# imkaywu/MVSKit

Measured on AMD Instinct MI355X. Metric: patches/s (propagate+optim iteration), 12-view 1080p, higher is better.
Workload: dtype f32

## Files before the change

mvskit_amd/csrc/mvs_engine.cpp:

```cpp
#include <hip/hip_runtime.h>
#include <dlfcn.h>
#include <rccl/rccl.h>

#include <algorithm>
#include <climits>
#include <cmath>
#include <cstdio>
#include <cstdlib>
#include <cstring>
#include <string>
#include <vector>

#include "mvskit_engine.h"
#include "mvs_kernels.h"
#include "mvs_types.h"

static_assert(sizeof(mvs_patch) == sizeof(DPatch), "mvs_patch and DPatch must be the same bytes");
static_assert((MVS_LISTCAP == 16 || MVS_LISTCAP == 32 || MVS_LISTCAP == 64) && MVS_LISTCAP <= MVS_MAXI && MVS_MAX_IMAGES == MVS_MAXI, "limits out of sync");

namespace {
thread_local std::string g_err;

#define HIPCHK(expr)                                                                                       \
    do {                                                                                                   \
        hipError_t _e = (expr);                                                                            \
        if (_e != hipSuccess) {                                                                            \
            g_err = std::string(#expr) + ": " + hipGetErrorString(_e);                                     \
            return MVS_ERR_HIP;                                                                            \
        }                                                                                                  \
    } while (0)

template <typename T> struct DevBuf {
    T* p = nullptr;
    int64_t cap = 0;
    bool headroom = false;
    DevBuf() = default;
    DevBuf(const DevBuf&) = delete;
    DevBuf(DevBuf&& o) noexcept : p(o.p), cap(o.cap), headroom(o.headroom) { o.p = nullptr; o.cap = 0; }
    ~DevBuf() { release(); }
    void swap(DevBuf& o) { std::swap(p, o.p); std::swap(cap, o.cap); }
    int ensure(int64_t n) {
        if (n <= cap) return MVS_OK;
        const int64_t exact = std::max<int64_t>(n, 16);
        int64_t want = (p && headroom) ? exact + exact / 2 : exact;
        T* q = nullptr;
        hipError_t e = hipMalloc((void**)&q, (size_t)want * sizeof(T));
        if (e != hipSuccess && want > exact) { (void)hipGetLastError(); want = exact; e = hipMalloc((void**)&q, (size_t)want * sizeof(T)); }
        if (e != hipSuccess && p) {
            (void)hipGetLastError();
            (void)hipFree(p); p = nullptr; cap = 0;
            e = hipMalloc((void**)&q, (size_t)want * sizeof(T));
        }
        if (e != hipSuccess) { (void)hipGetLastError(); g_err = std::string("hipMalloc: ") + hipGetErrorString(e); return MVS_ERR_HIP; }
        if (p) (void)hipFree(p);
        p = q; cap = want;
        return MVS_OK;
    }
    void release() { if (p) (void)hipFree(p); p = nullptr; cap = 0; }
};

namespace misc {
constexpr int stage_counter = 0;
constexpr int fill_evals = 1;
constexpr int neighbor_retry = 4;
constexpr int sweep_retry = 5;
constexpr int geo_bad = 6;
constexpr int group_edges = 7;
constexpr int trim_parts = 8;
constexpr int trim_nparts = 256;
constexpr int words = trim_parts + trim_nparts;
}
namespace fstat {
constexpr int neighbor_parts = 0;
constexpr int neighbor_cycles = 4096;
constexpr int exact_evals = 4112;
constexpr int words = exact_evals + 2048;
}

struct Rccl {
    void* h = nullptr;
    ncclResult_t (*GetUniqueId)(ncclUniqueId*) = nullptr;
    ncclResult_t (*CommInitRank)(ncclComm_t*, int, ncclUniqueId, int) = nullptr;
    ncclResult_t (*CommDestroy)(ncclComm_t) = nullptr;
    ncclResult_t (*CommCount)(const ncclComm_t, int*) = nullptr;
    ncclResult_t (*CommUserRank)(const ncclComm_t, int*) = nullptr;
    ncclResult_t (*AllGather)(const void*, void*, size_t, ncclDataType_t, ncclComm_t, hipStream_t) = nullptr;
    ncclResult_t (*Broadcast)(const void*, void*, size_t, ncclDataType_t, int, ncclComm_t, hipStream_t) = nullptr;
    ncclResult_t (*GroupStart)() = nullptr;
    ncclResult_t (*GroupEnd)() = nullptr;
    const char* (*GetErrorString)(ncclResult_t) = nullptr;
    bool ok = false;
};
Rccl& rccl() {
    static Rccl r;
    static bool tried = false;
    if (tried) return r;
    tried = true;
    if (const char* over = getenv("MVS_CCL_LIBRARY")) {
        if (*over) { r.h = dlopen(over, RTLD_NOW | RTLD_LOCAL); if (!r.h) return r; }
    }
    const char* names[] = {"librccl.so", "librccl.so.1"};
    for (const char* n : names) if (!r.h) r.h = dlopen(n, RTLD_NOW | RTLD_NOLOAD);
    const char* paths[] = {"/opt/rocm/lib/librccl.so.1", "librccl.so.1", "librccl.so"};
    for (const char* n : paths) if (!r.h) r.h = dlopen(n, RTLD_NOW | RTLD_LOCAL);
    if (!r.h) return r;
#define MVS_SYM(field, name) r.field = reinterpret_cast<decltype(r.field)>(dlsym(r.h, name))
    MVS_SYM(GetUniqueId, "ncclGetUniqueId"); MVS_SYM(CommInitRank, "ncclCommInitRank"); MVS_SYM(CommDestroy, "ncclCommDestroy");
    MVS_SYM(AllGather, "ncclAllGather"); MVS_SYM(Broadcast, "ncclBroadcast"); MVS_SYM(GroupStart, "ncclGroupStart");
    MVS_SYM(GroupEnd, "ncclGroupEnd"); MVS_SYM(GetErrorString, "ncclGetErrorString");
    MVS_SYM(CommCount, "ncclCommCount"); MVS_SYM(CommUserRank, "ncclCommUserRank");
#undef MVS_SYM
    r.ok = r.GetUniqueId && r.CommInitRank && r.CommDestroy && r.AllGather && r.Broadcast && r.GroupStart && r.GroupEnd && r.GetErrorString;
    return r;
}
#define NCCLCHK(expr)                                                                                      \
    do {                                                                                                   \
        ncclResult_t _r = (expr);                                                                          \
        if (_r != ncclSuccess) {                                                                           \
            g_err = std::string(#expr) + ": " + rccl().GetErrorString(_r);                                 \
            return MVS_ERR_HIP;                                                                            \
        }                                                                                                  \
    } while (0)

// ... 1006 lines not shown
    int64_t nj = 0;
    const bool ranged = e->cfg.shard_count > 1;
    for (int v = ranged ? 0 : e->cfg.view_begin; v < e->cfg.nviews; v += ranged ? 1 : e->cfg.view_stride) {
        a.sweep_views[a.nsweep_views] = v;
        a.job_base[a.nsweep_views] = (int32_t)nj;
        ++a.nsweep_views;
        nj += (int64_t)((e->hviews[v].gw + 1) / 2) * e->hviews[v].gh;
    }
    a.njobs = nj;
    a.job_lo = 0; a.job_hi = nj;
    if (ranged) {
        const int split_mode = getenv("MVS_SPLIT_PROXY") ? atoi(getenv("MVS_SPLIT_PROXY")) : 2;
        const int N = e->cfg.shard_count, R = e->cfg.shard_index;
        std::vector<int32_t> cuts(N + 1, -1);
        int64_t total_work = 0;
        if (split_mode > 0 && nj > 0) {
            const DParams p0 = current_params(e);
            int shift = 0;
            while ((((int64_t)3 * e->prm.cap * e->prm.max_propag * 32 * nj) >> shift) + nj >= (int64_t)INT32_MAX) ++shift;
            mvsk_job_work(p0, a, split_mode, shift, e->job_cnt.p, st);
            mvsk_exclusive_scan(e->job_cnt.p, e->job_base_scan.p, nj, reinterpret_cast<int32_t*>(e->scan_tmp.p), st);
            if (int r = e->tmp_i.ensure(N + 1)) return r;
            HIPCHK(hipMemsetAsync(e->tmp_i.p, 0xff, (size_t)(N + 1) * sizeof(int32_t), st));
            mvsk_job_cuts(e->job_base_scan.p, nj, N, e->tmp_i.p, st);
            int32_t tw = 0;
            HIPCHK(hipMemcpyAsync(cuts.data(), e->tmp_i.p, (size_t)(N + 1) * sizeof(int32_t), hipMemcpyDeviceToHost, st));
            HIPCHK(hipMemcpyAsync(&tw, e->job_base_scan.p + nj, sizeof tw, hipMemcpyDeviceToHost, st));
            HIPCHK(hipStreamSynchronize(st));
            total_work = tw;
        }
        cuts[0] = 0; cuts[N] = (int32_t)nj;
        for (int r = 1; r < N; ++r) {
            if (total_work <= 0 || cuts[r] < 0) cuts[r] = (int32_t)(nj * r / N);
            cuts[r] = std::max(cuts[r], cuts[r - 1]);
        }
        a.job_lo = cuts[R];
        a.job_hi = cuts[R + 1];
        HIPCHK(hipMemsetAsync(e->job_nstage.p, 0, (size_t)nj * sizeof(int32_t), st));
    }
    a.staging = e->staging.p; a.staging_cap = e->staging.cap;
    a.stage_counter = e->misc.p + misc::stage_counter;
    a.job_stage = e->job_stage.p; a.job_nstage = e->job_nstage.p;
    a.maxstage = (e->prm.view_propagation ? 3 : 2) * e->prm.cap * e->prm.max_propag;
    a.kill = e->kill.p;
    a.counters = e->counters.p;
    a.error_flag = e->error_flag.p;
    if (want_vgrid(e)) {
        if (int r = e->big_tables.ensure((int64_t)256 * 16384)) return r;
        if (int r = e->retry_jobs.ensure(std::max<int64_t>(nj, 16))) return r;
    }
    a.big_tables = e->big_tables.p; a.retry_jobs = e->retry_jobs.p; a.nretry = reinterpret_cast<int32_t*>(e->misc.p + misc::sweep_retry);
    HIPCHK(hipMemsetAsync(e->misc.p + misc::sweep_retry, 0, sizeof(unsigned long long), st));
    HIPCHK(hipMemsetAsync(e->misc.p + misc::stage_counter, 0, sizeof(unsigned long long), st));
    HIPCHK(hipMemsetAsync(e->counters.p, 0, MVS_COUNTER_SLOTS * sizeof(DCounters), st));
    HIPCHK(hipMemsetAsync(e->error_flag.p, 0, sizeof(int32_t), st));
    const DParams p = current_params(e);
    const RefineSel rs = refine_sel(e);
    mvsk_sweep(p, a, rs, st);
    e->pass_retried = 0;
    if (want_vgrid(e)) {
        int32_t nretry = 0;
        HIPCHK(hipMemcpyAsync(&nretry, a.nretry, sizeof nretry, hipMemcpyDeviceToHost, st));
        HIPCHK(hipStreamSynchronize(st));
        e->pass_retried = nretry;
        if (nretry > 0) { mvsk_sweep_retry(p, a, nretry, rs, st); e->retried_cells += nretry; }
    }
    HIPCHK(hipEventRecord(e->ev[2], st));
    std::vector<DCounters> hcs(MVS_COUNTER_SLOTS);
    int32_t herr = 0;
    unsigned long long fill[2] = {0, 0};
    HIPCHK(hipMemcpyAsync(fill, e->misc.p + misc::fill_evals, sizeof fill, hipMemcpyDeviceToHost, st));
    HIPCHK(hipMemcpyAsync(hcs.data(), e->counters.p, hcs.size() * sizeof(DCounters), hipMemcpyDeviceToHost, st));
    HIPCHK(hipMemcpyAsync(&herr, e->error_flag.p, sizeof herr, hipMemcpyDeviceToHost, st));
    HIPCHK(hipStreamSynchronize(st));
    HIPCHK(hipGetLastError());
    mvs_counters sum{};
    for (const DCounters& c : hcs) add_counters(sum, c);
    sum.evals += fill[0]; sum.view_evals += fill[1]; sum.trimmed = (int64_t)trimmed;
    float ms = 0.0f;
    (void)hipEventElapsedTime(&ms, e->ev[0], e->ev[1]); e->timing.index_ms = ms;
    (void)hipEventElapsedTime(&ms, e->ev[1], e->ev[2]); e->timing.sweep_ms = ms;
    e->timing.commit_ms = 0.0f; e->timing.sweep_launches = 1; e->timing.exchange_ms = 0.0f; e->timing.exchange_bytes = 0;
    e->timing.check_retried_cells = e->pass_retried;
    e->staged = true; e->counted = false;
    if (out) *out = sum;
#ifdef MVS_STAGE_TIMING
    {
        unsigned long long stage[16] = {0};
        for (const DCounters& c : hcs)
            for (int k = 0; k < 16; ++k) stage[k] = (k == 12 || k == 13) ? std::max(stage[k], c.stage[k]) : stage[k] + c.stage[k];
        static const char* nm[8] = {"wave", "generate", "pre", "refine", "post", "check", "stage", "prologue"};
        fprintf(stderr, "[stage cycles]");
        for (int k = 0; k < 8; ++k) fprintf(stderr, " %s %.1f%%", nm[k], 100.0 * (double)stage[k] / (double)(stage[0] ? stage[0] : 1));
        static const char* nm2[4] = {"gain", "search", "sort", "quad"};
        for (int k = 0; k < 4; ++k) fprintf(stderr, " %s %.1f%%", nm2[k], 100.0 * (double)stage[8 + k] / (double)(stage[0] ? stage[0] : 1));
        fprintf(stderr, " setRefImage pairs %.1f%% choice %.1f%%", 100.0 * (double)stage[14] / (double)(stage[0] ? stage[0] : 1), 100.0 * (double)stage[15] / (double)(stage[0] ? stage[0] : 1));
        fprintf(stderr, "  (wave cycles %.3e; max visited %llu, max neighbours %llu)\n", (double)stage[0], stage[12], stage[13]);
    }
#endif
#ifdef MVS_FAULT_INJECTION
    if (const char* f = getenv("MVS_FAULT_PASS")) {
        int fr = -1, fi = -1, fp = -1;
        if (!e->fault_fired && sscanf(f, "%d:%d:%d", &fr, &fi, &fp) == 3 && fr == (e->cfg.shard_count > 1 ? e->cfg.shard_index : 0) && fi == iter && fp == pass) {
            e->fault_fired = true;
            g_err = "mvs_engine_pass: capacity failure injected by MVS_FAULT_PASS";
            return MVS_ERR_CAPACITY;
// ... 450 lines not shown
```

mvskit_amd/csrc/mvs_kernels.hip:

```cpp
#include <hip/hip_runtime.h>
#include <algorithm>
#include "mvs_device.cuh"
#include "mvs_check.cuh"
#include "mvs_kernels.h"

using namespace mvsdev;

__global__ void k_rgb_to_rgba(const uint8_t* __restrict__ rgb, uint32_t* __restrict__ out, int64_t n) {
    const int64_t i = (int64_t)blockIdx.x * blockDim.x + threadIdx.x;
    if (i >= n) return;
    const uint8_t* p = rgb + 3 * i;
    out[i] = (uint32_t)p[0] | ((uint32_t)p[1] << 8) | ((uint32_t)p[2] << 16);
}
__global__ void k_rgba_to_rgb(const uint32_t* __restrict__ in, uint8_t* __restrict__ rgb, int64_t n) {
    const int64_t i = (int64_t)blockIdx.x * blockDim.x + threadIdx.x;
    if (i >= n) return;
    const uint32_t t = in[i];
    rgb[3 * i] = t & 255u; rgb[3 * i + 1] = (t >> 8) & 255u; rgb[3 * i + 2] = (t >> 16) & 255u;
}
__global__ void k_pyr_down(const uint32_t* __restrict__ src, int pw, int ph, uint32_t* __restrict__ dst, int w, int h) {
    const int x = blockIdx.x * blockDim.x + threadIdx.x, y = blockIdx.y * blockDim.y + threadIdx.y;
    if (x >= w || y >= h) return;
    const float base[4] = {1.0f, 3.0f, 3.0f, 1.0f};
    float c0 = 0.0f, c1 = 0.0f, c2 = 0.0f;
// ... 255 lines not shown
    int ix, iy;
    cell_of(prm, vw, ld4(p->coord), ix, iy);
    if (ix < 0 || vw->gw <= ix || iy < 0 || vw->gh <= iy) return;
    const unsigned long long key = ((unsigned long long)sortable_f32(p->ncc) << 32) | (unsigned long long)(0xffffffffu - (uint32_t)id);
    atomicMax(&best[iy * vw->gw + ix], key);
}
__global__ void k_map_extract(DParams prm, int view, int kind, const unsigned long long* __restrict__ sel, float* __restrict__ depth,
                              float* __restrict__ normal, int32_t* __restrict__ ids, int ncells) {
    const int c = blockIdx.x * blockDim.x + threadIdx.x;
    if (c >= ncells) return;
    const unsigned long long k = sel[c];
    const bool empty = kind == 0 ? (k == ~0ull) : (k == 0ull);
    if (empty) {
        depth[c] = __int_as_float(0x7fc00000);
        normal[3 * c] = normal[3 * c + 1] = normal[3 * c + 2] = __int_as_float(0x7fc00000);
        ids[c] = -1;
        return;
    }
    const uint32_t id = kind == 0 ? (uint32_t)(k & 0xffffffffull) : 0xffffffffu - (uint32_t)(k & 0xffffffffull);
    const DPatch* p = prm.pool + id;
    depth[c] = dot4(ld4((prm.views + view)->oaxis), ld4(p->coord));
    normal[3 * c] = p->normal[0]; normal[3 * c + 1] = p->normal[1]; normal[3 * c + 2] = p->normal[2];
    ids[c] = (int32_t)id;
}

__global__ __launch_bounds__(64) void k_fill_ncc(DParams prm, unsigned long long* evals) {
    WaveCtx wc = make_wave_ctx(prm);
    const int64_t mine = (int64_t)blockIdx.x * 64 + wc.lane;
    bool need = false;
    if (mine < prm.pool_n) need = (prm.pool[mine].flags & 1) && (prm.pool[mine].ncc < 0.0f);
    unsigned long long todo = ballot(need);
    while (todo) {
        const int l = __ffsll((long long)todo) - 1;
        todo &= todo - 1ull;
        DPatch* p = prm.pool + ((int64_t)blockIdx.x * 64 + l);
        Cand c;
        load_cand(p, wc, c);
        const float ncc = compute_ncc(prm, wc, c.coord, c.normal, c.img, c.nimg);
        if (wc.lane == 0) p->ncc = ncc;
    }
    if (wc.lane == 0 && wc.evals) { atomicAdd(evals, (unsigned long long)wc.evals); atomicAdd(evals + 1, (unsigned long long)wc.view_evals); }
}

DEV bool rank_before(float na, int a, float nb, int b) { return (na != nb) ? (na > nb) : (a < b); }
DEV void job_cell(const DParams& prm, const SweepArgs& a, int64_t job, int& v, int& cx, int& cy) {
    int s = 0;
    while (s + 1 < a.nsweep_views && job >= a.job_base[s + 1]) ++s;
    v = a.sweep_views[s];
    const int gw = (prm.views + v)->gw, halfw = (gw + 1) / 2;
    const int local = (int)(job - a.job_base[s]);
    cy = local / halfw;
    cx = 2 * (local % halfw) + ((a.colour + cy) & 1);
}
__global__ void k_job_work(DParams prm, SweepArgs a, int mode, int shift, int32_t* __restrict__ work) {
    const int64_t job = (int64_t)blockIdx.x * blockDim.x + threadIdx.x;
    if (job >= a.njobs) return;
    int v, cx, cy;
    job_cell(prm, a, job, v, cx, cy);
    const DView* vw = prm.views + v;
    const int gw = vw->gw, gh = vw->gh;
    int w = 0;
    if (cx < gw && cy < gh) {
        const int sxs[3] = {cx, cx - a.inc, cx}, sys[3] = {cy - a.inc, cy, cy};
        const int nsrc = prm.view_propagation ? 3 : 2;
        int n = 0;
        for (int k = 0; k < nsrc; ++k) {
            if (sxs[k] < 0 || gw <= sxs[k] || sys[k] < 0 || gh <= sys[k]) continue;
            const int g = vw->cell_base + sys[k] * gw + sxs[k];
            const csr_off_t sb = prm.csr_start[g];
            const int sn = prm.csr_cnt[g];
            for (int j = 0; j < sn; ++j) n += ((pgrid_ref(prm, sb + j) == v) != (k == 2)) ? 1 : 0;
        }
        if (mode == 1) w = n;
        else {
            const int trials = n * prm.max_propag;
            const int room = max(prm.cap - prm.csr_cnt[vw->cell_base + cy * gw + cx], 0);
            const int full = min(trials, (room * 5 + 3) / 4);
            w = 32 * full + 2 * (trials - full);
        }
    }
    work[job] = (w + (1 << shift) - 1) >> shift;
}
__global__ void k_job_cuts(const int32_t* __restrict__ scan, int64_t njobs, int n, int32_t* __restrict__ cuts) {
    const int64_t job = (int64_t)blockIdx.x * blockDim.x + threadIdx.x;
    if (job >= njobs) return;
    const long long total = scan[njobs], p0 = scan[job], p1 = scan[job + 1];
    if (p0 == p1) return;
    for (int r = 1; r < n; ++r) {
        const long long target = total * r / n;
        if (p0 <= target && target < p1) cuts[r] = (int32_t)job;
    }
}

#ifndef MVS_SWEEP_WAVES
#define MVS_SWEEP_WAVES 3
#endif
#ifdef MVS_STAGE_TIMING
#define ST_NOW() ((unsigned long long)__builtin_amdgcn_s_memtime())
#define ST_ADD(k, t0) { const unsigned long long t1_ = ST_NOW(); st_acc[k] += t1_ - (t0); (t0) = t1_; }
#else
#define ST_ADD(k, t0)
#endif
#ifndef MVS_XCD_CHUNK
#define MVS_XCD_CHUNK 128
#endif
template <bool BIG, bool SIMPLEX = false>
DEV void sweep_cell(const DParams& prm, const SweepArgs& a, const int64_t job, int* s_scratch, float* s_texs, int* big_table,
                    int max_evals = 0, float xtol = 0.0f) {
#ifdef MVS_STAGE_TIMING
    unsigned long long st_acc[16] = {0, 0, 0, 0, 0, 0, 0, 0, 0, 0, 0, 0, 0, 0, 0, 0};
    const unsigned long long st_begin = ST_NOW();
    unsigned long long st_t = st_begin;
#endif
    int v, cx, cy;
    job_cell(prm, a, job, v, cx, cy);
    const DView* vw = prm.views + v;
    const int gw = vw->gw, gh = vw->gh;
    WaveCtx wc = make_wave_ctx(prm);
    if (wc.lane == 0) a.job_nstage[job] = 0;
    if (cx >= gw || cy >= gh) return;
    const int cell = cy * gw + cx;
    const int inc = a.inc;
    const int sxs[2] = {cx, cx - inc}, sys[2] = {cy - inc, cy};
    bool has = false;
    for (int k = 0; k < 2; ++k) {
        if (sxs[k] < 0 || gw <= sxs[k] || sys[k] < 0 || gh <= sys[k]) continue;
        const int g = vw->cell_base + sys[k] * gw + sxs[k];
        has |= prm.csr_cnt[g] > 0;
    }
    if (prm.view_propagation) has |= prm.csr_cnt[vw->cell_base + cy * gw + cx] > 0;
    if (!has) return;

    const int tstride = prm.wsz;
    unsigned n_cand = 0, n_pref = 0, n_patch = 0, n_f0 = 0, n_f1 = 0, n_ins = 0, n_rep = 0;
    int L_id = -1;
    float L_ncc = 0.0f;
    int L_n = 0;
    {
        const int g = vw->cell_base + cell;
        const csr_off_t fb = prm.csr_start[g];
        L_n = min(prm.csr_cnt[g], MVS_CAPMAX);
        if (wc.lane < L_n) { L_id = pgrid_id(prm, fb + wc.lane); L_ncc = pgrid_ncc(prm, fb + wc.lane); }
    }
    int ns = 0;
    bool gave_up = false;
    const float icx = (float)(prm.csize * (2 * cx + 1) - 1) / 2.0f, icy = (float)(prm.csize * (2 * cy + 1) - 1) / 2.0f;

    const int nsrc = prm.view_propagation ? 3 : 2;
    for (int sidx = 0; sidx < nsrc; ++sidx) {
        const int scx = sidx < 2 ? sxs[sidx] : cx, scy = sidx < 2 ? sys[sidx] : cy;
        if (scx < 0 || gw <= scx || scy < 0 || gh <= scy) continue;
        const int g = vw->cell_base + scy * gw + scx;
        const csr_off_t sb = prm.csr_start[g];
        const int sn = min(prm.csr_cnt[g], MVS_CAPMAX);
        const int as_view = sidx == 2 ? v : -1;
        int E_id = 0;
        bool E_take = false;
        if (wc.lane < sn) { E_id = pgrid_id(prm, sb + wc.lane); E_take = (pgrid_ref(prm, sb + wc.lane) == v) != (sidx == 2); }
        unsigned todo = (unsigned)ballot(E_take);
        while (todo) {
            const int n = __ffs((int)todo) - 1;
            todo &= todo - 1u;
            const DPatch* sp = prm.pool + rli(E_id, n);
            const int srcslot = sidx * prm.cap + n;
            for (int it = 0; it < prm.max_propag; ++it) {
                ST_ADD(7, st_t)
                const int np = L_n;
                const uint32_t k0 = (uint32_t)a.iter, k1 = (uint32_t)v, k2 = (uint32_t)cell, k3 = (uint32_t)(srcslot * 16 + it);
                Cand c;
                int worst = -1;
                float worst_ncc = 0.0f;
                F3 ic;
                if (np < prm.cap) {
                    const float ra = rng_uniform(prm.seed, k0, k1, k2, k3, 0) * (float)prm.csize;
                    const float rb = rng_uniform(prm.seed, k0, k1, k2, k3, 1) * (float)prm.csize;
                    ic = {icx + ra, icy + rb, 1.0f};
                } else {
                    worst = rli(L_id, prm.cap - 1);
                    worst_ncc = rlf(L_ncc, prm.cap - 1);
                    const DPatch* wp = worst >= MVS_NEWBASE ? a.staging + (worst - MVS_NEWBASE) : prm.pool + worst;
                    ic = project(vw, ld4(wp->coord), prm.level);
                }
                {
                    Cand src;
// ... 17 lines not shown
                if (post_r == -1) { ++n_f1; continue; }
                if (prm.depth >= 2 && prm.enable_check) {
                    __syncthreads();
                    if (wc.lane < MVS_CAPMAX) s_scratch[wc.lane] = L_id;
                    __syncthreads();
                    #ifdef MVS_STAGE_TIMING
                    const CheckCtx cx{a.staging, v, cell, L_n, s_scratch, st_acc};
#else
                    const CheckCtx cx{a.staging, v, cell, L_n, s_scratch, nullptr};
#endif
                    const int chk_r = check_patch<BIG>(prm, wc, cx, c, s_texs, a.error_flag, big_table);
                    ST_ADD(5, st_t)
                    if (!BIG && chk_r < 0) { gave_up = true; break; }
                    if (chk_r) { ++n_f1; continue; }
                }
                unsigned long long slot64 = 0;
                if (wc.lane == 0) slot64 = atomicAdd(a.stage_counter, 1ull);
                const int64_t slot = ((int64_t)rfl((int)(slot64 >> 32)) << 32) | (uint32_t)rfl((int)(slot64 & 0xffffffffull));
                if (slot >= a.staging_cap || ns >= a.maxstage) {
                    if (wc.lane == 0) atomicOr(a.error_flag, 1);
                    continue;
                }
                if (np == prm.cap) {
                    if (wc.lane == 0) {
                        if (worst >= MVS_NEWBASE) a.staging[worst - MVS_NEWBASE].flags &= ~1;
                        else a.kill[worst] = 1;
                    }
                    --L_n;
                    ++n_rep;
                } else ++n_ins;
                store_cand(a.staging + slot, wc, c, 1 | (v << 8), cell);
                if (wc.lane == 0) a.job_stage[job * a.maxstage + ns] = (int32_t)slot;
                ++ns;
                const bool lands = ballot(wc.lane < c.nimg && c.img == v && c.gy * gw + c.gx == cell) != 0ull;
                if (lands) {
                    const int nid = MVS_NEWBASE + (int)slot;
                    const int pos = __popcll(ballot(wc.lane < L_n && rank_before(L_ncc, L_id, c.ncc, nid)));
                    const int up_id = __shfl_up(L_id, 1);
                    const float up_ncc = __shfl_up(L_ncc, 1);
                    if (wc.lane > pos) { L_id = up_id; L_ncc = up_ncc; }
                    if (wc.lane == pos) { L_id = nid; L_ncc = c.ncc; }
                    ++L_n;
                }
                ST_ADD(6, st_t)
            }
            if (gave_up) break;
        }
        if (gave_up) break;
    }
    if (!BIG && gave_up) {
        if (wc.lane == 0) { a.job_nstage[job] = 0; a.retry_jobs[atomicAdd(a.nretry, 1)] = (int32_t)job; }
        return;
    }
    if (wc.lane == 0) {
        a.job_nstage[job] = ns;
        DCounters* C = a.counters + (job & (MVS_COUNTER_SLOTS - 1));
        if (n_cand) atomicAdd(&C->candidates, (unsigned long long)n_cand);
        if (n_pref) atomicAdd(&C->prefiltered, (unsigned long long)n_pref);
        if (n_patch) atomicAdd(&C->patches, (unsigned long long)n_patch);
        if (n_f0) atomicAdd(&C->fail0, (unsigned long long)n_f0);
        if (n_f1) atomicAdd(&C->fail1, (unsigned long long)n_f1);
        if (n_ins) atomicAdd(&C->inserted, (unsigned long long)n_ins);
        if (n_rep) atomicAdd(&C->replaced, (unsigned long long)n_rep);
        if (wc.evals) atomicAdd(&C->evals, (unsigned long long)wc.evals);
        if (wc.view_evals) atomicAdd(&C->view_evals, (unsigned long long)wc.view_evals);
#ifdef MVS_STAGE_TIMING
        st_acc[0] = ST_NOW() - st_begin;
        for (int k = 0; k < 12; ++k) if (st_acc[k]) atomicAdd(&C->stage[k], st_acc[k]);
        atomicMax(&C->stage[12], st_acc[12]); atomicMax(&C->stage[13], st_acc[13]);
        atomicAdd(&C->stage[14], wc.st_acc[3]); atomicAdd(&C->stage[15], wc.st_acc[4]);
#endif
    }
}

DEV int64_t sweep_job(const SweepArgs& a) {
    const int64_t bi = blockIdx.x >> 3;
    const int64_t job = a.job_lo + (bi / MVS_XCD_CHUNK) * (8 * MVS_XCD_CHUNK) + (int64_t)(blockIdx.x & 7u) * MVS_XCD_CHUNK + (bi % MVS_XCD_CHUNK);
    return job;
}
__global__ __launch_bounds__(64, MVS_SWEEP_WAVES) void k_sweep(DParams prm, SweepArgs a) {
    __shared__ int s_scratch[192];
    extern __shared__ float s_texs[];
    const int64_t bi = blockIdx.x >> 3;
    const int64_t job = a.job_lo + (bi / MVS_XCD_CHUNK) * (8 * MVS_XCD_CHUNK) + (int64_t)(blockIdx.x & 7u) * MVS_XCD_CHUNK + (bi % MVS_XCD_CHUNK);
    if (job >= a.job_hi) return;
    sweep_cell<false>(prm, a, job, s_scratch, s_texs, nullptr);
}
__global__ __launch_bounds__(64, MVS_SWEEP_WAVES) void k_sweep_simplex(DParams prm, SweepArgs a, int max_evals, float xtol) {
    __shared__ int s_scratch[192];
    extern __shared__ float s_texs[];
    const int64_t job = sweep_job(a);
    if (job >= a.job_hi) return;
    sweep_cell<false, true>(prm, a, job, s_scratch, s_texs, nullptr, max_evals, xtol);
}
__global__ __launch_bounds__(64, 1) void k_sweep_retry(DParams prm, SweepArgs a, int nretry) {
    __shared__ int s_scratch[192];
    extern __shared__ float s_texs[];
    int* big_table = a.big_tables + (size_t)blockIdx.x * MVS_FILTER2_HASH_CAP;
    for (int k = blockIdx.x; k < nretry; k += gridDim.x) {
        __syncthreads();
        sweep_cell<true>(prm, a, (int64_t)a.retry_jobs[k], s_scratch, s_texs, big_table);
    }
}
__global__ __launch_bounds__(64, 1) void k_sweep_retry_simplex(DParams prm, SweepArgs a, int nretry, int max_evals, float xtol) {
    __shared__ int s_scratch[192];
    extern __shared__ float s_texs[];
    int* big_table = a.big_tables + (size_t)blockIdx.x * MVS_FILTER2_HASH_CAP;
    for (int k = blockIdx.x; k < nretry; k += gridDim.x) {
        __syncthreads();
        sweep_cell<true, true>(prm, a, (int64_t)a.retry_jobs[k], s_scratch, s_texs, big_table, max_evals, xtol);
    }
}

__global__ void k_commit_count(SweepArgs a, int32_t* __restrict__ cnt) {
    const int64_t job = (int64_t)blockIdx.x * blockDim.x + threadIdx.x;
    if (job >= a.njobs) return;
    const int ns = a.job_nstage[job];
    int c = 0;
    for (int k = 0; k < ns; ++k) c += a.staging[a.job_stage[job * a.maxstage + k]].flags & 1;
    cnt[job] = c;
}
__global__ void k_commit_copy(SweepArgs a, const int32_t* __restrict__ base, DPatch* __restrict__ dst, int64_t dst_cap, int32_t* __restrict__ per_view,
                              int keep_key) {
    const int64_t job = (int64_t)blockIdx.x * blockDim.x + threadIdx.x;
    if (job >= a.njobs) return;
    const int ns = a.job_nstage[job];
    int r = 0;
    for (int k = 0; k < ns; ++k) {
        const DPatch* sp = a.staging + a.job_stage[job * a.maxstage + k];
        if (!(sp->flags & 1)) continue;
        const int64_t o = (int64_t)base[job] + r++;
        if (o >= dst_cap) { atomicOr(a.error_flag, 2); return; }
        const uint4* s4 = reinterpret_cast<const uint4*>(sp);
        uint4* d4 = reinterpret_cast<uint4*>(dst + o);
        for (int w = 0; w < (int)MVS_REC_U4; ++w) d4[w] = s4[w];
        if (per_view) atomicAdd(&per_view[(sp->flags >> 8) & 0xff], 1);
        if (!keep_key) { dst[o].flags = 1; dst[o].id = 0; }
    }
}
__global__ void k_kill_count(const uint8_t* __restrict__ kill, int64_t n, int32_t* __restrict__ cnt) {
    const int64_t i = (int64_t)blockIdx.x * blockDim.x + threadIdx.x;
    if (i < n) cnt[i] = kill[i] ? 1 : 0;
}
__global__ void k_kill_export(const uint8_t* __restrict__ kill, int64_t n, const int32_t* __restrict__ base, int32_t* __restrict__ ids, int64_t cap) {
    const int64_t i = (int64_t)blockIdx.x * blockDim.x + threadIdx.x;
    if (i < n && kill[i] && base[i] < cap) ids[base[i]] = (int32_t)i;
}
__global__ void k_apply_kill_flags(DPatch* pool, uint8_t* kill, int64_t n) {
    const int64_t i = (int64_t)blockIdx.x * blockDim.x + threadIdx.x;
    if (i < n && kill[i]) { pool[i].flags &= ~1; kill[i] = 0; }
}
__global__ void k_apply_kill_ids(DPatch* pool, const int32_t* __restrict__ ids, int64_t n, int64_t pool_n) {
    const int64_t i = (int64_t)blockIdx.x * blockDim.x + threadIdx.x;
    if (i < n && ids[i] >= 0 && ids[i] < pool_n) pool[ids[i]].flags &= ~1;
}
__global__ void k_append_records(DPatch* pool, int64_t pool_n, const DPatch* __restrict__ recs, int64_t n) {
    const int64_t i = (int64_t)blockIdx.x * blockDim.x + threadIdx.x;
    if (i >= n) return;
    const uint4* s4 = reinterpret_cast<const uint4*>(recs + i);
    uint4* d4 = reinterpret_cast<uint4*>(pool + pool_n + i);
    for (int w = 0; w < (int)MVS_REC_U4; ++w) d4[w] = s4[w];
    pool[pool_n + i].flags = 1;
    pool[pool_n + i].id = 0;
// ... 458 lines not shown
void mvsk_mask_binarise(uint8_t* m, int64_t n, hipStream_t st) { hipLaunchKernelGGL(k_mask_binarise, dim3(nblk(n, 256)), dim3(256), 0, st, m, n); }
void mvsk_exclusive_scan(const int32_t* in, int32_t* out, int64_t n, int32_t* tmp, hipStream_t st) { launch_exclusive_scan<int32_t, int32_t>(in, out, n, tmp, st); }
void mvsk_exclusive_scan_off(const int32_t* in, csr_off_t* out, int64_t n, csr_off_t* tmp, hipStream_t st) { launch_exclusive_scan<int32_t, csr_off_t>(in, out, n, tmp, st); }
void mvsk_index_count(const DParams& prm, int32_t* cnt, int32_t* vcnt, unsigned long long* total, hipStream_t st) {
    if (prm.pool_n > 0) hipLaunchKernelGGL(k_index_count, dim3(nblk(prm.pool_n, 256)), dim3(256), 0, st, prm, cnt, vcnt, total);
}
void mvsk_index_fill(const DParams& prm, int vgrid, const csr_off_t* start, int32_t* cursor, unsigned long long* ids, hipStream_t st) {
    if (prm.pool_n > 0) hipLaunchKernelGGL(k_index_fill, dim3(nblk(prm.pool_n, 256)), dim3(256), 0, st, prm, vgrid, start, cursor, ids);
}
void mvsk_index_fill_direct(const DParams& prm, int vgrid, const csr_off_t* start, int32_t* cursor, int32_t* id32, hipStream_t st) {
    if (prm.pool_n > 0) hipLaunchKernelGGL(k_index_fill_direct, dim3(nblk(prm.pool_n, 256)), dim3(256), 0, st, prm, vgrid, start, cursor, id32);
}
void mvsk_index_sort_trim(const DParams& prm, const csr_off_t* start, unsigned long long* ids, int do_trim, unsigned long long* trimmed, hipStream_t st) {
    hipLaunchKernelGGL(k_index_sort_trim, dim3(nblk(prm.total_cells, 256)), dim3(256), 0, st, prm, start, ids, do_trim, trimmed);
}
void mvsk_index_finalize(const DParams& prm, int vgrid, const csr_off_t* start, unsigned long long* ids, int32_t* id32, int32_t* cnt_alive, hipStream_t st) {
    hipLaunchKernelGGL(k_index_finalize, dim3(nblk(prm.total_cells, 256)), dim3(256), 0, st, prm, vgrid, start, ids, id32, cnt_alive);
}
void mvsk_index_pack(const DParams& prm, const csr_off_t* start, const csr_off_t* start2, const int32_t* cnt_alive, const unsigned long long* ids, const int32_t* id32_in,
                     ListKey* key, int32_t* id32_out, hipStream_t st) {
    hipLaunchKernelGGL(k_index_pack, dim3(nblk(prm.total_cells, 256)), dim3(256), 0, st, prm, start, start2, cnt_alive, ids, id32_in, key, id32_out);
}
void mvsk_depth_maps(const DParams& prm, unsigned long long* dp, const uint32_t* dirty, hipStream_t st) {
    if (prm.pool_n > 0) hipLaunchKernelGGL(k_depth_maps, dim3(nblk(prm.pool_n, 64)), dim3(256), 0, st, prm, dp, dirty);
}
void mvsk_depth_mark_dirty(const DParams& prm, const uint8_t* kill, unsigned long long* dp, uint32_t* dirty, hipStream_t st) {
    if (prm.pool_n > 0) hipLaunchKernelGGL(k_depth_mark_dirty, dim3(nblk(prm.pool_n, 64)), dim3(256), 0, st, prm, kill, dp, dirty);
}
void mvsk_best_ncc_map(const DParams& prm, int view, unsigned long long* best, hipStream_t st) {
    if (prm.pool_n > 0) hipLaunchKernelGGL(k_best_ncc_map, dim3(nblk(prm.pool_n, 256)), dim3(256), 0, st, prm, view, best);
}
void mvsk_map_extract(const DParams& prm, int view, int kind, const unsigned long long* sel, float* depth, float* normal, int32_t* ids, int ncells, hipStream_t st) {
    hipLaunchKernelGGL(k_map_extract, dim3(nblk(ncells, 256)), dim3(256), 0, st, prm, view, kind, sel, depth, normal, ids, ncells);
}
void mvsk_fill_ncc(const DParams& prm, unsigned long long* evals, hipStream_t st) {
    if (prm.pool_n > 0) hipLaunchKernelGGL(k_fill_ncc, dim3((unsigned)((prm.pool_n + 63) / 64)), dim3(64), MVS_FRAME_LDS_BYTES, st, prm, evals);
}
size_t mvsk_sweep_lds_bytes(const DParams& prm) {
#if MVS_PAIR_MFMA
    const size_t tex_f = (size_t)MVS_GRAM_CH * 3 * prm.wsz, gram_f = (size_t)prm.gram_ld * prm.gram_ld;
    const size_t texs = MVS_FRAME1_LDS_BYTES + (tex_f > gram_f ? tex_f : gram_f) * sizeof(float);
#else
    const size_t ln = (size_t)prm.list_n;
    const size_t texs = MVS_FRAME1_LDS_BYTES + (ln * 3 * prm.wsz + ln * (ln - 1) / 2) * sizeof(float);
#endif
    const size_t chk = (size_t)MVS_CHECK_LDS_FLOATS * sizeof(float);
    const size_t need = texs > chk ? texs : chk;
    return need > (size_t)MVS_FRAME_LDS_BYTES ? need : (size_t)MVS_FRAME_LDS_BYTES;
}
void mvsk_sweep(const DParams& prm, const SweepArgs& a, const RefineSel& rs, hipStream_t st) {
    const int64_t nloc = a.job_hi - a.job_lo;
    if (nloc <= 0) return;
    static const size_t pad = getenv("MVS_SWEEP_LDS_PAD") ? (size_t)atol(getenv("MVS_SWEEP_LDS_PAD")) : 0;
    const int64_t nblocks = (nloc + 8 * MVS_XCD_CHUNK - 1) / (8 * MVS_XCD_CHUNK) * (8 * MVS_XCD_CHUNK);
    if (rs.simplex) hipLaunchKernelGGL(k_sweep_simplex, dim3((unsigned)nblocks), dim3(64), mvsk_sweep_lds_bytes(prm) + pad, st, prm, a, rs.max_evals, rs.xtol);
    else hipLaunchKernelGGL(k_sweep, dim3((unsigned)nblocks), dim3(64), mvsk_sweep_lds_bytes(prm) + pad, st, prm, a);
}
void mvsk_job_work(const DParams& prm, const SweepArgs& a, int mode, int shift, int32_t* work, hipStream_t st) {
    if (a.njobs > 0) hipLaunchKernelGGL(k_job_work, dim3(nblk(a.njobs, 256)), dim3(256), 0, st, prm, a, mode, shift, work);
}
void mvsk_job_cuts(const int32_t* scan, int64_t njobs, int n, int32_t* cuts, hipStream_t st) {
    if (njobs > 0) hipLaunchKernelGGL(k_job_cuts, dim3(nblk(njobs, 256)), dim3(256), 0, st, scan, njobs, n, cuts);
}
void mvsk_sweep_retry(const DParams& prm, const SweepArgs& a, int nretry, const RefineSel& rs, hipStream_t st) {
    if (nretry <= 0) return;
    const dim3 grid((unsigned)std::min(nretry, MVS_BIG_SLOTS));
    if (rs.simplex) hipLaunchKernelGGL(k_sweep_retry_simplex, grid, dim3(64), mvsk_sweep_lds_bytes(prm), st, prm, a, nretry, rs.max_evals, rs.xtol);
    else hipLaunchKernelGGL(k_sweep_retry, grid, dim3(64), mvsk_sweep_lds_bytes(prm), st, prm, a, nretry);
}
void mvsk_commit_count(const SweepArgs& a, int32_t* cnt, hipStream_t st) { hipLaunchKernelGGL(k_commit_count, dim3(nblk(a.njobs, 256)), dim3(256), 0, st, a, cnt); }
void mvsk_commit_copy(const SweepArgs& a, const int32_t* base, DPatch* dst, int64_t dst_cap, int32_t* per_view, int keep_key, hipStream_t st) {
    hipLaunchKernelGGL(k_commit_copy, dim3(nblk(a.njobs, 256)), dim3(256), 0, st, a, base, dst, dst_cap, per_view, keep_key);
}
void mvsk_kill_count(const uint8_t* kill, int64_t n, int32_t* cnt, hipStream_t st) { if (n > 0) hipLaunchKernelGGL(k_kill_count, dim3(nblk(n, 256)), dim3(256), 0, st, kill, n, cnt); }
void mvsk_kill_export(const uint8_t* kill, int64_t n, const int32_t* base, int32_t* ids, int64_t cap, hipStream_t st) {
    if (n > 0) hipLaunchKernelGGL(k_kill_export, dim3(nblk(n, 256)), dim3(256), 0, st, kill, n, base, ids, cap);
}
void mvsk_apply_kill_flags(DPatch* pool, uint8_t* kill, int64_t n, hipStream_t st) { if (n > 0) hipLaunchKernelGGL(k_apply_kill_flags, dim3(nblk(n, 256)), dim3(256), 0, st, pool, kill, n); }
void mvsk_apply_kill_ids(DPatch* pool, const int32_t* ids, int64_t n, int64_t pool_n, hipStream_t st) {
    if (n > 0) hipLaunchKernelGGL(k_apply_kill_ids, dim3(nblk(n, 256)), dim3(256), 0, st, pool, ids, n, pool_n);
}
void mvsk_append_records(DPatch* pool, int64_t pool_n, const DPatch* recs, int64_t n, hipStream_t st) {
    if (n > 0) hipLaunchKernelGGL(k_append_records, dim3(nblk(n, 256)), dim3(256), 0, st, pool, pool_n, recs, n);
}
void mvsk_alive_count(const DPatch* pool, int64_t n, int32_t* cnt, hipStream_t st) { if (n > 0) hipLaunchKernelGGL(k_alive_count, dim3(nblk(n, 256)), dim3(256), 0, st, pool, n, cnt); }
void mvsk_alive_gather(const DPatch* pool, int64_t n, const int32_t* base, DPatch* out, int64_t cap, hipStream_t st) {
    if (n > 0) hipLaunchKernelGGL(k_alive_gather, dim3(nblk(n, 256)), dim3(256), 0, st, pool, n, base, out, cap);
}
void mvsk_filter_vimages(const DParams& prm, int additive, int64_t first, int64_t last, const uint32_t* dirty, hipStream_t st) {
    if (last <= first) return;
    const int gl = std::max(prm.nviews <= 16 ? 16 : (prm.nviews <= 32 ? 32 : 64), (int)MVS_LISTCAP);
    const unsigned nb = (unsigned)((last - first + 64 / gl - 1) / (64 / gl));
    if (gl == 16) hipLaunchKernelGGL(k_filter_vimages<16>, dim3(nb), dim3(64), 0, st, prm, additive, first, last, dirty);
    else if (gl == 32) hipLaunchKernelGGL(k_filter_vimages<32>, dim3(nb), dim3(64), 0, st, prm, additive, first, last, dirty);
    else hipLaunchKernelGGL(k_filter_vimages<64>, dim3(nb), dim3(64), 0, st, prm, additive, first, last, dirty);
}
void mvsk_geo_pack(const DPatch* pool, int64_t n, float4* geo, uint8_t* ref, int* bad, hipStream_t st) {
    if (n <= 0) return;
    hipLaunchKernelGGL(k_geo_pack, dim3((unsigned)((n + 255) / 256)), dim3(256), 0, st, pool, n, geo, ref, bad);
}
void mvsk_filter_outside(const DParams& prm, uint8_t* kill, int64_t first, int64_t last, hipStream_t st) {
    if (last > first) hipLaunchKernelGGL(k_filter_outside, dim3((unsigned)(last - first)), dim3(64), 0, st, prm, kill, first);
}
size_t mvsk_texs_lds_bytes(const DParams& prm) {
#if MVS_PAIR_MFMA
    const size_t tex_f = (size_t)MVS_GRAM_CH * 3 * prm.wsz, gram_f = (size_t)prm.gram_ld * prm.gram_ld;
    const size_t texs = MVS_FRAME1_LDS_BYTES + (tex_f > gram_f ? tex_f : gram_f) * sizeof(float);
#else
    const size_t ln = (size_t)prm.list_n;
// ... 54 lines not shown
```

mvskit_amd/csrc/mvs_types.h:

```cpp
#pragma once
#include <stdint.h>

#define MVS_WAVE 64
#define MVS_MAXLEV 7
#ifndef MVS_LISTCAP
#define MVS_LISTCAP 16
#endif
#if MVS_LISTCAP > 32
#define MVS_MAXI 64
#else
#define MVS_MAXI 32
#endif
#define MVS_MAXVIEWS 64
#define MVS_CAPMAX 32
#define MVS_NEWBASE 0x40000000

#define MVS_FLAG_ALIVE 1
#define MVS_FLAG_SETTLED 2
struct DPatch {
    float coord[4];
    float normal[4];
    float ncc, dscale, ascale, tmp;
    int32_t nimages, nvimages, flags, id;
    uint8_t images[MVS_MAXI];
// ... 4 lines not shown

typedef int64_t csr_off_t;
struct ListKey {
    float ncc;
    int32_t ref;
};
static_assert(sizeof(ListKey) == 8, "list key is 8 bytes");

struct DView {
    float P[MVS_MAXLEV][12];
    float Minv[9];
    float center[4];
    float oaxis[4];
    float xaxis[3], yaxis[3], zaxis[3];
    float ipscale;
    int32_t W[MVS_MAXLEV], H[MVS_MAXLEV];
    const uint32_t* img[MVS_MAXLEV];
    const uint8_t* mask;
    int32_t gw, gh;
    int32_t cell_base;
    int32_t pad;
};

struct DParams {
    int32_t nviews, level, csize, wsize, wsz, minImageNum, tau, cap, max_propag, depth, enable_check, view_propagation;
    uint32_t seed;
    int32_t refine_steps;
    float rd0, ra0;
    float nccThreshold, nccThresholdBefore;
    float cosAngle0, cosAngle1, cosMinAngle, cosMaxAngle, cosNeighborTypo, cosNeighbor120;
    float sortThreshold, ascaleConst, neighborThreshold, neighborThreshold1, quadThreshold;
    float inv_sz, inv_3sz;
    int32_t total_cells;
    int32_t list_n;
    int32_t gram_ld;
    const DView* views;
    DPatch* pool;
    int64_t pool_n;
    const csr_off_t* csr_start;
    const int32_t* csr_cnt;
    const ListKey* csr_key;
    const int32_t* csr_id32;
    const csr_off_t* vcsr_start;
    const int32_t* vcsr_cnt;
    const int32_t* vcsr_id32;
    const float4* geo;
    const uint8_t* geo_ref;
    const unsigned long long* dpgrid;
};

#ifndef MVS_COUNTER_SLOTS
#define MVS_COUNTER_SLOTS 256
#endif
struct DCounters {
    unsigned long long candidates, prefiltered, patches, fail0, fail1, inserted, replaced, evals, view_evals, trimmed;
    unsigned long long stage[16];
};

struct SweepArgs {
    int32_t iter, inc, colour;
    int32_t nsweep_views;
    int32_t sweep_views[MVS_MAXVIEWS];
    int32_t job_base[MVS_MAXVIEWS];
    int32_t halfw_max, gh_max;
    int64_t njobs;
    int64_t job_lo, job_hi;
    DPatch* staging;
    int64_t staging_cap;
    unsigned long long* stage_counter;
    int32_t* job_stage;
    int32_t* job_nstage;
    int32_t maxstage;
    uint8_t* kill;
    DCounters* counters;
    int32_t* error_flag;
    int32_t* big_tables;
    int32_t* retry_jobs;
    int32_t* nretry;
};
```

Before: 27.89 million.

## Replace one-block-per-cell sweep with persistent blocks pulling jobs from per-XCD queues

The sweep kernel now launches a grid sized to the device (CUs × 4 × waves) instead of one block per job. Each persistent wave pulls job ranges from eight atomic cursor queues that mirror the old XCD chunk mapping, and a wave-wide ballot skips cells with no source patches before any heavy work. Counter atomics are accumulated in registers per wave and flushed once at the end instead of after every cell. This is meant to cut launch and block-scheduling overhead for empty cells and to reduce global atomic traffic, at the cost of atomic cursor contention and possible load imbalance across persistent blocks.

```diff
diff --git a/mvskit_amd/csrc/mvs_engine.cpp b/mvskit_amd/csrc/mvs_engine.cpp
--- a/mvskit_amd/csrc/mvs_engine.cpp
+++ b/mvskit_amd/csrc/mvs_engine.cpp
@@ -68,7 +68,9 @@
 constexpr int group_edges = 7;
 constexpr int trim_parts = 8;
 constexpr int trim_nparts = 256;
-constexpr int words = trim_parts + trim_nparts;
+constexpr int sweep_cursors = (trim_parts + trim_nparts + 15) / 16 * 16;
+constexpr int sweep_cursor_words = MVS_SWEEP_QUEUES * MVS_SWEEP_CURSOR_STRIDE * (int)sizeof(uint32_t) / (int)sizeof(unsigned long long);
+constexpr int words = sweep_cursors + sweep_cursor_words;
 }
 namespace fstat {
 constexpr int neighbor_parts = 0;
@@ -1181,6 +1183,8 @@
     a.big_tables = e->big_tables.p; a.retry_jobs = e->retry_jobs.p; a.nretry = reinterpret_cast<int32_t*>(e->misc.p + misc::sweep_retry);
     HIPCHK(hipMemsetAsync(e->misc.p + misc::sweep_retry, 0, sizeof(unsigned long long), st));
     HIPCHK(hipMemsetAsync(e->misc.p + misc::stage_counter, 0, sizeof(unsigned long long), st));
+    a.cursors = reinterpret_cast<uint32_t*>(e->misc.p + misc::sweep_cursors);
+    HIPCHK(hipMemsetAsync(e->misc.p + misc::sweep_cursors, 0, misc::sweep_cursor_words * sizeof(unsigned long long), st));
     HIPCHK(hipMemsetAsync(e->counters.p, 0, MVS_COUNTER_SLOTS * sizeof(DCounters), st));
     HIPCHK(hipMemsetAsync(e->error_flag.p, 0, sizeof(int32_t), st));
     const DParams p = current_params(e);
diff --git a/mvskit_amd/csrc/mvs_kernels.hip b/mvskit_amd/csrc/mvs_kernels.hip
--- a/mvskit_amd/csrc/mvs_kernels.hip
+++ b/mvskit_amd/csrc/mvs_kernels.hip
@@ -331,6 +331,22 @@
     cy = local / halfw;
     cx = 2 * (local % halfw) + ((a.colour + cy) & 1);
 }
+DEV bool job_has_source(const DParams& prm, const SweepArgs& a, int64_t job) {
+    int v, cx, cy;
+    job_cell(prm, a, job, v, cx, cy);
+    const DView* vw = prm.views + v;
+    const int gw = vw->gw, gh = vw->gh;
+    if (cx >= gw || cy >= gh) return false;
+    const int sxs[2] = {cx, cx - a.inc}, sys[2] = {cy - a.inc, cy};
+    bool has = false;
+    for (int k = 0; k < 2; ++k) {
+        if (sxs[k] < 0 || gw <= sxs[k] || sys[k] < 0 || gh <= sys[k]) continue;
+        const int g = vw->cell_base + sys[k] * gw + sxs[k];
+        has |= prm.csr_cnt[g] > 0;
+    }
+    if (prm.view_propagation) has |= prm.csr_cnt[vw->cell_base + cy * gw + cx] > 0;
+    return has;
+}
 __global__ void k_job_work(DParams prm, SweepArgs a, int mode, int shift, int32_t* __restrict__ work) {
     const int64_t job = (int64_t)blockIdx.x * blockDim.x + threadIdx.x;
     if (job >= a.njobs) return;
@@ -383,32 +399,56 @@
 #ifndef MVS_XCD_CHUNK
 #define MVS_XCD_CHUNK 128
 #endif
+struct SweepAcc {
+    unsigned cand, pref, patch, f0, f1, ins, rep;
+    unsigned long long evals, view_evals;
+#ifdef MVS_STAGE_TIMING
+    unsigned long long stage[16];
+#endif
+};
+DEV SweepAcc sweep_acc_zero() {
+    SweepAcc acc;
+    acc.cand = acc.pref = acc.patch = acc.f0 = acc.f1 = acc.ins = acc.rep = 0u;
+    acc.evals = acc.view_evals = 0ull;
+#ifdef MVS_STAGE_TIMING
+    for (int k = 0; k < 16; ++k) acc.stage[k] = 0ull;
+#endif
+    return acc;
+}
+DEV void sweep_acc_flush(const SweepArgs& a, const SweepAcc& acc, unsigned slot) {
+    DCounters* C = a.counters + slot;
+    if (acc.cand) atomicAdd(&C->candidates, (unsigned long long)acc.cand);
+    if (acc.pref) atomicAdd(&C->prefiltered, (unsigned long long)acc.pref);
+    if (acc.patch) atomicAdd(&C->patches, (unsigned long long)acc.patch);
+    if (acc.f0) atomicAdd(&C->fail0, (unsigned long long)acc.f0);
+    if (acc.f1) atomicAdd(&C->fail1, (unsigned long long)acc.f1);
+    if (acc.ins) atomicAdd(&C->inserted, (unsigned long long)acc.ins);
+    if (acc.rep) atomicAdd(&C->replaced, (unsigned long long)acc.rep);
+    if (acc.evals) atomicAdd(&C->evals, acc.evals);
+    if (acc.view_evals) atomicAdd(&C->view_evals, acc.view_evals);
+#ifdef MVS_STAGE_TIMING
+    for (int k = 0; k < 12; ++k) if (acc.stage[k]) atomicAdd(&C->stage[k], acc.stage[k]);
+    atomicMax(&C->stage[12], acc.stage[12]); atomicMax(&C->stage[13], acc.stage[13]);
+    atomicAdd(&C->stage[14], acc.stage[14]); atomicAdd(&C->stage[15], acc.stage[15]);
+#endif
+}
 template <bool BIG, bool SIMPLEX = false>
-DEV void sweep_cell(const DParams& prm, const SweepArgs& a, const int64_t job, int* s_scratch, float* s_texs, int* big_table,
-                    int max_evals = 0, float xtol = 0.0f) {
+DEV void sweep_cell(const DParams& prm, const SweepArgs& a, WaveCtx& wc, SweepAcc* acc, const int64_t job, int* s_scratch, float* s_texs,
+                    int* big_table, int max_evals = 0, float xtol = 0.0f) {
 #ifdef MVS_STAGE_TIMING
     unsigned long long st_acc[16] = {0, 0, 0, 0, 0, 0, 0, 0, 0, 0, 0, 0, 0, 0, 0, 0};
     const unsigned long long st_begin = ST_NOW();
     unsigned long long st_t = st_begin;
+    for (int k = 0; k < 8; ++k) wc.st_acc[k] = 0;
 #endif
     int v, cx, cy;
     job_cell(prm, a, job, v, cx, cy);
     const DView* vw = prm.views + v;
     const int gw = vw->gw, gh = vw->gh;
-    WaveCtx wc = make_wave_ctx(prm);
-    if (wc.lane == 0) a.job_nstage[job] = 0;
-    if (cx >= gw || cy >= gh) return;
+    wc.evals = 0; wc.view_evals = 0;
     const int cell = cy * gw + cx;
     const int inc = a.inc;
     const int sxs[2] = {cx, cx - inc}, sys[2] = {cy - inc, cy};
-    bool has = false;
-    for (int k = 0; k < 2; ++k) {
-        if (sxs[k] < 0 || gw <= sxs[k] || sys[k] < 0 || gh <= sys[k]) continue;
-        const int g = vw->cell_base + sys[k] * gw + sxs[k];
-        has |= prm.csr_cnt[g] > 0;
-    }
-    if (prm.view_propagation) has |= prm.csr_cnt[vw->cell_base + cy * gw + cx] > 0;
-    if (!has) return;
 
     const int tstride = prm.wsz;
     unsigned n_cand = 0, n_pref = 0, n_patch = 0, n_f0 = 0, n_f1 = 0, n_ins = 0, n_rep = 0;
@@ -532,46 +572,71 @@
         if (wc.lane == 0) { a.job_nstage[job] = 0; a.retry_jobs[atomicAdd(a.nretry, 1)] = (int32_t)job; }
         return;
     }
-    if (wc.lane == 0) {
-        a.job_nstage[job] = ns;
-        DCounters* C = a.counters + (job & (MVS_COUNTER_SLOTS - 1));
-        if (n_cand) atomicAdd(&C->candidates, (unsigned long long)n_cand);
-        if (n_pref) atomicAdd(&C->prefiltered, (unsigned long long)n_pref);
-        if (n_patch) atomicAdd(&C->patches, (unsigned long long)n_patch);
-        if (n_f0) atomicAdd(&C->fail0, (unsigned long long)n_f0);
-        if (n_f1) atomicAdd(&C->fail1, (unsigned long long)n_f1);
-        if (n_ins) atomicAdd(&C->inserted, (unsigned long long)n_ins);
-        if (n_rep) atomicAdd(&C->replaced, (unsigned long long)n_rep);
-        if (wc.evals) atomicAdd(&C->evals, (unsigned long long)wc.evals);
-        if (wc.view_evals) atomicAdd(&C->view_evals, (unsigned long long)wc.view_evals);
+    if (wc.lane == 0) a.job_nstage[job] = ns;
+    {
+        acc->cand += n_cand; acc->pref += n_pref; acc->patch += n_patch; acc->f0 += n_f0; acc->f1 += n_f1; acc->ins += n_ins; acc->rep += n_rep;
+        acc->evals += wc.evals; acc->view_evals += wc.view_evals;
 #ifdef MVS_STAGE_TIMING
         st_acc[0] = ST_NOW() - st_begin;
-        for (int k = 0; k < 12; ++k) if (st_acc[k]) atomicAdd(&C->stage[k], st_acc[k]);
-        atomicMax(&C->stage[12], st_acc[12]); atomicMax(&C->stage[13], st_acc[13]);
-        atomicAdd(&C->stage[14], wc.st_acc[3]); atomicAdd(&C->stage[15], wc.st_acc[4]);
-#endif
-    }
-}
-
-DEV int64_t sweep_job(const SweepArgs& a) {
-    const int64_t bi = blockIdx.x >> 3;
-    const int64_t job = a.job_lo + (bi / MVS_XCD_CHUNK) * (8 * MVS_XCD_CHUNK) + (int64_t)(blockIdx.x & 7u) * MVS_XCD_CHUNK + (bi % MVS_XCD_CHUNK);
-    return job;
+        for (int k = 0; k < 12; ++k) acc->stage[k] += st_acc[k];
+        acc->stage[12] = max(acc->stage[12], st_acc[12]); acc->stage[13] = max(acc->stage[13], st_acc[13]);
+        acc->stage[14] += wc.st_acc[3]; acc->stage[15] += wc.st_acc[4];
+#endif
+    }
+}
+
+#ifndef MVS_SWEEP_TAKE
+#define MVS_SWEEP_TAKE 1
+#endif
+static_assert(MVS_SWEEP_TAKE <= 64 && MVS_XCD_CHUNK % MVS_SWEEP_TAKE == 0, "a take is a part of one chunk, a lane per job");
+template <bool SIMPLEX>
+DEV void sweep_resident(const DParams& prm, const SweepArgs& a, int* s_scratch, float* s_texs, int max_evals, float xtol) {
+    WaveCtx wc = make_wave_ctx(prm);
+    SweepAcc acc = sweep_acc_zero();
+    const int nchunks = (int)((a.job_hi - a.job_lo + MVS_XCD_CHUNK - 1) / MVS_XCD_CHUNK);
+    constexpr unsigned per = MVS_XCD_CHUNK / MVS_SWEEP_TAKE;
+    for (unsigned step = 0; step < MVS_SWEEP_QUEUES; ++step) {
+        const unsigned q = (blockIdx.x + step) & (MVS_SWEEP_QUEUES - 1u);
+        const unsigned ntake = (unsigned)((nchunks - (int)q + MVS_SWEEP_QUEUES - 1) / MVS_SWEEP_QUEUES) * per;
+        for (;;) {
+            unsigned k = 0;
+            if (wc.lane == 0) k = atomicAdd(a.cursors + q * MVS_SWEEP_CURSOR_STRIDE, 1u);
+            k = (unsigned)rfl((int)k);
+            if (k >= ntake) break;
+            const int64_t base = a.job_lo + ((int64_t)q + (int64_t)MVS_SWEEP_QUEUES * (k / per)) * MVS_XCD_CHUNK + (int64_t)(k % per) * MVS_SWEEP_TAKE;
+            const int64_t mine = base + wc.lane;
+            bool has = false;
+            if (wc.lane < MVS_SWEEP_TAKE && mine < a.job_hi) {
+                a.job_nstage[mine] = 0;
+                has = job_has_source(prm, a, mine);
+            }
+            unsigned long long t = ballot(has);
+            while (t) {
+                const int l = __ffsll((long long)t) - 1;
+                t &= t - 1ull;
+                __syncthreads();
+                sweep_cell<false, SIMPLEX>(prm, a, wc, &acc, base + l, s_scratch, s_texs, nullptr, max_evals, xtol);
+            }
+        }
+    }
+    if (wc.lane == 0) sweep_acc_flush(a, acc, blockIdx.x & (MVS_COUNTER_SLOTS - 1));
 }
 __global__ __launch_bounds__(64, MVS_SWEEP_WAVES) void k_sweep(DParams prm, SweepArgs a) {
     __shared__ int s_scratch[192];
     extern __shared__ float s_texs[];
-    const int64_t bi = blockIdx.x >> 3;
-    const int64_t job = a.job_lo + (bi / MVS_XCD_CHUNK) * (8 * MVS_XCD_CHUNK) + (int64_t)(blockIdx.x & 7u) * MVS_XCD_CHUNK + (bi % MVS_XCD_CHUNK);
-    if (job >= a.job_hi) return;
-    sweep_cell<false>(prm, a, job, s_scratch, s_texs, nullptr);
+    sweep_resident<false>(prm, a, s_scratch, s_texs, 0, 0.0f);
 }
 __global__ __launch_bounds__(64, MVS_SWEEP_WAVES) void k_sweep_simplex(DParams prm, SweepArgs a, int max_evals, float xtol) {
     __shared__ int s_scratch[192];
     extern __shared__ float s_texs[];
-    const int64_t job = sweep_job(a);
-    if (job >= a.job_hi) return;
-    sweep_cell<false, true>(prm, a, job, s_scratch, s_texs, nullptr, max_evals, xtol);
+    sweep_resident<true>(prm, a, s_scratch, s_texs, max_evals, xtol);
+}
+template <bool SIMPLEX>
+DEV void sweep_retry_cell(const DParams& prm, const SweepArgs& a, const int64_t job, int* s_scratch, float* s_texs, int* big_table, int max_evals, float xtol) {
+    WaveCtx wc = make_wave_ctx(prm);
+    SweepAcc acc = sweep_acc_zero();
+    sweep_cell<true, SIMPLEX>(prm, a, wc, &acc, job, s_scratch, s_texs, big_table, max_evals, xtol);
+    if (wc.lane == 0) sweep_acc_flush(a, acc, (unsigned)(job & (MVS_COUNTER_SLOTS - 1)));
 }
 __global__ __launch_bounds__(64, 1) void k_sweep_retry(DParams prm, SweepArgs a, int nretry) {
     __shared__ int s_scratch[192];
@@ -579,7 +644,7 @@
     int* big_table = a.big_tables + (size_t)blockIdx.x * MVS_FILTER2_HASH_CAP;
     for (int k = blockIdx.x; k < nretry; k += gridDim.x) {
         __syncthreads();
-        sweep_cell<true>(prm, a, (int64_t)a.retry_jobs[k], s_scratch, s_texs, big_table);
+        sweep_retry_cell<false>(prm, a, (int64_t)a.retry_jobs[k], s_scratch, s_texs, big_table, 0, 0.0f);
     }
 }
 __global__ __launch_bounds__(64, 1) void k_sweep_retry_simplex(DParams prm, SweepArgs a, int nretry, int max_evals, float xtol) {
@@ -588,7 +653,7 @@
     int* big_table = a.big_tables + (size_t)blockIdx.x * MVS_FILTER2_HASH_CAP;
     for (int k = blockIdx.x; k < nretry; k += gridDim.x) {
         __syncthreads();
-        sweep_cell<true, true>(prm, a, (int64_t)a.retry_jobs[k], s_scratch, s_texs, big_table, max_evals, xtol);
+        sweep_retry_cell<true>(prm, a, (int64_t)a.retry_jobs[k], s_scratch, s_texs, big_table, max_evals, xtol);
     }
 }
 
@@ -1153,9 +1218,18 @@
     const int64_t nloc = a.job_hi - a.job_lo;
     if (nloc <= 0) return;
     static const size_t pad = getenv("MVS_SWEEP_LDS_PAD") ? (size_t)atol(getenv("MVS_SWEEP_LDS_PAD")) : 0;
-    const int64_t nblocks = (nloc + 8 * MVS_XCD_CHUNK - 1) / (8 * MVS_XCD_CHUNK) * (8 * MVS_XCD_CHUNK);
-    if (rs.simplex) hipLaunchKernelGGL(k_sweep_simplex, dim3((unsigned)nblocks), dim3(64), mvsk_sweep_lds_bytes(prm) + pad, st, prm, a, rs.max_evals, rs.xtol);
-    else hipLaunchKernelGGL(k_sweep, dim3((unsigned)nblocks), dim3(64), mvsk_sweep_lds_bytes(prm) + pad, st, prm, a);
+    const size_t lds = mvsk_sweep_lds_bytes(prm) + pad;
+    int dev = 0, cus = 0;
+    (void)hipGetDevice(&dev);
+    if (hipDeviceGetAttribute(&cus, hipDeviceAttributeMultiprocessorCount, dev) != hipSuccess || cus <= 0) { (void)hipGetLastError(); cus = 256; }
+    int64_t nblocks = (int64_t)cus * 4 * MVS_SWEEP_WAVES;
+    nblocks = std::min(nblocks, (nloc + MVS_SWEEP_TAKE - 1) / MVS_SWEEP_TAKE);
+    if (const char* g = getenv("MVS_SWEEP_GRID")) {
+        const long cap = atol(g);
+        if (cap > 0) nblocks = std::min<int64_t>(nblocks, cap);
+    }
+    if (rs.simplex) hipLaunchKernelGGL(k_sweep_simplex, dim3((unsigned)nblocks), dim3(64), lds, st, prm, a, rs.max_evals, rs.xtol);
+    else hipLaunchKernelGGL(k_sweep, dim3((unsigned)nblocks), dim3(64), lds, st, prm, a);
 }
 void mvsk_job_work(const DParams& prm, const SweepArgs& a, int mode, int shift, int32_t* work, hipStream_t st) {
     if (a.njobs > 0) hipLaunchKernelGGL(k_job_work, dim3(nblk(a.njobs, 256)), dim3(256), 0, st, prm, a, mode, shift, work);
diff --git a/mvskit_amd/csrc/mvs_types.h b/mvskit_amd/csrc/mvs_types.h
--- a/mvskit_amd/csrc/mvs_types.h
+++ b/mvskit_amd/csrc/mvs_types.h
@@ -80,6 +80,8 @@
 #ifndef MVS_COUNTER_SLOTS
 #define MVS_COUNTER_SLOTS 256
 #endif
+#define MVS_SWEEP_QUEUES 8
+#define MVS_SWEEP_CURSOR_STRIDE 32
 struct DCounters {
     unsigned long long candidates, prefiltered, patches, fail0, fail1, inserted, replaced, evals, view_evals, trimmed;
     unsigned long long stage[16];
@@ -105,4 +107,5 @@
     int32_t* big_tables;
     int32_t* retry_jobs;
     int32_t* nretry;
+    uint32_t* cursors;
 };
```

Result: faster. 28.89 million, median of 6 (+3.6%).
